# YonghaoHe/LFD-A-Light-and-Fast-Detector

Hardware: AMD Instinct MI355X
Metric: images/sec WIDERFACE-S 1920x1080 bs=8 end-to-end inference, LFD.precision='fp32_storage' (raw logits within 1e-4 of fp32: inside north_star's 1e-3; the 'fp16' mode, sigma 2.5e-3, under fp16_mode) (higher is better)
Workload: dtype f16

## Files before the change

### include/lfd_hip.h

```cpp
#ifndef LFD_HIP_H_
#define LFD_HIP_H_

#include <stddef.h>
#include <stdint.h>

#ifdef __cplusplus
extern "C" {
#endif

#define LFD_HIP_ABI_VERSION 3
#define LFD_MAX_LEVELS 8

typedef void* lfd_stream_t;

#if defined(LFD_BUILDING)
#define LFD_API __attribute__((visibility("default")))
#else
#define LFD_API
#endif

enum lfd_status {
  LFD_OK = 0,
  LFD_ERR_INVALID_ARGUMENT = -1,
  LFD_ERR_WORKSPACE_TOO_SMALL = -2,
// ... 204 lines not shown
                                              int32_t w, int32_t c, lfd_stream_t stream);
LFD_API int lfd_relu_inplace_f16(void* x, int64_t count, lfd_stream_t stream);
LFD_API int lfd_maxpool3x3s2_nhwc_f16(const void* in, void* out, int32_t n, int32_t h, int32_t w, int32_t c,
                                      lfd_stream_t stream);
LFD_API int lfd_pack_level_outputs_f32(const float* src, float* dst, int32_t n, int32_t hw, int32_t src_channels, int32_t c0,
                                       int32_t count, int32_t total_points, int32_t point_offset, float scale, int32_t op,
                                       lfd_stream_t stream);

LFD_API int lfd_conv2d_nhwc_f16_acc32(const lfd_conv_desc_t* desc, const void* in, float* out_f32, const void* w_packed,
                                      const float* bias, const void* zeros, lfd_stream_t stream);

typedef struct lfd_p32_conv_desc {
  int32_t n, h, w, cin, cout, ks, stride, relu;
  int32_t in_format;
  int32_t out_pixel_stride;
  int64_t out_image_stride;
} lfd_p32_conv_desc_t;
LFD_API size_t lfd_p32_conv_packed_weight_halfs(int32_t cin, int32_t cout, int32_t ks);
LFD_API int lfd_p32_conv2d_nhwc_f32(const lfd_p32_conv_desc_t* desc, const void* in, float* out, const void* w_packed,
                                    const float* bias, const float* residual, const float* scale, lfd_stream_t stream);
LFD_API int lfd_p32_conv2d_tail_nhwc_f32(const lfd_p32_conv_desc_t* desc, const void* in, float* out, const void* w_packed,
                                         const float* bias, const void* tail_w_packed, const float* tail_bias, int32_t tail_relu,
                                         lfd_stream_t stream);
LFD_API size_t lfd_p32_groupnorm_workspace_bytes(int32_t n, int32_t groups);
LFD_API int lfd_p32_groupnorm_relu_f32(float* x, int32_t n, int64_t hw, int32_t c, int32_t groups, const float* gamma,
                                       const float* beta, float eps, int32_t relu, void* workspace, size_t workspace_bytes,
                                       lfd_stream_t stream);

#define LFD_PL_GN_REPLICAS 8
typedef struct lfd_pl_conv_desc {
  int32_t n, h, w, cin, cout, ks, stride, relu;
  int32_t tail_cout, tail_relu;
  int32_t out_mode;
  int32_t f_c0, f_c1;
  float gn_in_eps;
  int64_t in_plane_halfs, out_plane_halfs, res_plane_halfs, ds_plane_halfs;
  int64_t f_image_stride0, f_image_stride1;
} lfd_pl_conv_desc_t;
LFD_API int lfd_pl_stem_pair(const void* in, int32_t in_format, int32_t n, int32_t h, int32_t w, int32_t channels,
                             const void* w1_packed, const float* b1, const void* w2_packed, const float* b2, void* out,
                             int64_t out_plane_halfs, lfd_stream_t stream);
LFD_API int lfd_pl_stem2x(const void* in, int32_t in_format, int32_t n, int32_t h, int32_t w, const void* w1_packed,
                          const void* w2_packed, const float* b2, const void* w3_packed, const float* b3,
                          const void* w4_packed, const float* b4, void* out, int64_t out_plane_halfs, const void* zeros,
                          lfd_stream_t stream);
LFD_API int lfd_pl_conv2d(const lfd_pl_conv_desc_t* desc, const void* in, void* out, const void* w_packed, const float* bias,
                          const void* residual, const void* tail_w_packed, const float* tail_bias, const void* ds_w_packed,
                          const float* ds_bias, void* ds_out, void* gn_sums, float* f_out0, float* f_out1, const float* scale1,
                          const void* gn_in_sums, const float* gn_in_gamma, const float* gn_in_beta, const void* zeros,
                          lfd_stream_t stream);
LFD_API int lfd_pl_block64(int32_t n, int32_t h, int32_t w, const void* in, int64_t in_plane_halfs, void* out,
                           int64_t out_plane_halfs, const void* w1_packed, const float* b1, const void* w2_packed,
                           const float* b2, const void* zeros, lfd_stream_t stream);
typedef struct lfd_pl_level {
  const void* in;
  void* out;
  const void* w_packed;
  const float* bias;
  const void* tail_w_packed;
  const float* tail_bias;
  void* gn_sums;
  const void* gn_in_sums;
  const float* gn_in_gamma;
  const float* gn_in_beta;
  float* f_out0;
  float* f_out1;
  const float* scale1;
  int32_t h, w;
  int64_t in_plane_halfs, out_plane_halfs;
} lfd_pl_level_t;
LFD_API int lfd_pl_conv2d_levels(const lfd_pl_conv_desc_t* desc, const lfd_pl_level_t* levels, int32_t num_levels,
                                 const void* zeros, lfd_stream_t stream);
LFD_API int lfd_pl_groupnorm_relu(void* x, int64_t plane_halfs, int32_t n, int64_t hw, int32_t c, const void* gn_sums,
                                  const float* gamma, const float* beta, float eps, int32_t relu, lfd_stream_t stream);

typedef struct lfd_pl_head_desc {
  int32_t mode, n, cin, relu0;
  int32_t f_c0, f_c1;
  float gn_in_eps;
  int32_t pad_;
  int64_t f_image_stride0, f_image_stride1;
} lfd_pl_head_desc_t;
typedef struct lfd_pl_head_level {
  const void* in;
  void* out;
  const void* w0;
  const float* b0;
  const void* w1;
  const float* b1;
  void* gn_sums;
  const void* gn_in_sums;
  const float* gn_in_gamma;
  const float* gn_in_beta;
  float* f_out0;
  float* f_out1;
  const float* scale1;
  int64_t in_plane_halfs;
  int32_t pixels, pad_;
} lfd_pl_head_level_t;
LFD_API int lfd_pl_head_levels(const lfd_pl_head_desc_t* desc, const lfd_pl_head_level_t* levels, int32_t num_levels,
                               const void* zeros, lfd_stream_t stream);

LFD_API int lfd_stem_conv_f16(const void* in, int32_t in_format, int32_t n, int32_t h, int32_t w,
                              int32_t channels, const void* w1_packed, const float* b1,
                              const void* w2_packed, const float* b2, void* out, lfd_stream_t stream);

// ... 232 lines not shown
```

### lfd-a-light-and-fast-detector_amd/lfd_amd/_lib.py

```python
import ctypes as C
import os

_HERE = os.path.dirname(os.path.abspath(__file__))
LIB_PATH = os.environ.get('LFD_HIP_LIB') or os.path.join(_HERE, 'liblfd_hip.so')
MAX_LEVELS = 8
F32, F16 = 0, 1

_lib = None


class DetectDesc(C.Structure):
    _fields_ = [('num_levels', C.c_int32),
                ('level_h', C.c_int32 * MAX_LEVELS), ('level_w', C.c_int32 * MAX_LEVELS),
                ('level_stride', C.c_int32 * MAX_LEVELS),
                ('level_range_lo', C.c_float * MAX_LEVELS), ('level_range_hi', C.c_float * MAX_LEVELS),
                ('num_classes', C.c_int32), ('num_cls_channels', C.c_int32),
                ('score_mode', C.c_int32), ('decode_mode', C.c_int32),
                ('class_agnostic', C.c_int32), ('max_candidates', C.c_int32),
                ('score_thr', C.c_float), ('iou_thr', C.c_float)]


class DetectExt(C.Structure):
    _fields_ = [('pre_nms_limit', C.c_int32), ('post_nms_limit', C.c_int32)]

# ... 175 lines not shown
    'lfd_gn_train_apply_f16': (C.c_int, [_P, _I32, _I64, _I32, _I32, _P, _P, _P, _I32, _P, _P]),
    'lfd_gn_train_stats_apply_f16': (C.c_int, [_P, _I32, _I64, _I32, _I32, _F, _P, _P, _I32, _P, _SZ, _P, _P, _P]),
    'lfd_gn_train_stats_apply_seg_f16': (C.c_int, [_P, _I32, _I32, _P, _I32, _I32, _F, _P, _P, _I32, _P, _SZ, _P, _P, _P]),
    'lfd_gn_train_bwd_seg_f16': (C.c_int, [_P, _P, _P, _I32, _I32, _P, _I32, _I32, _P, _P, _F, _I32, _P, _SZ, _P, _P, _P, _P]),
    'lfd_bn_train_apply_into_f16': (C.c_int, [_P, _I32, _I64, _I32, _P, _P, _P, _I32, _P, _I64, _I64, _P]),
    'lfd_bn_train_bwd_from_f16': (C.c_int, [_P, _I64, _I64, _P, _I32, _I32, _I64, _I32, _P, _P, _P, _F, _I32, _P, _SZ, _P, _P, _P, _P]),
    'lfd_head_out_split_concat_f16': (C.c_int, [_P, _I32, _I32, _I64, _I64, C.POINTER(HeadOutSeg), _I32, _P]),
    'lfd_head_out_grad_concat_f16': (C.c_int, [_P, _I32, _I32, _I64, _I64, C.POINTER(HeadOutSeg), _I32, _F, _P, _P, _SZ, _P]),
    'lfd_conv2d_bn_partials_nhwc_f16': (C.c_int, [C.POINTER(ConvDesc), _P, _P, _P, _P, _P, _P, _SZ, C.POINTER(C.c_int32), _P]),
    'lfd_bn_train_finish_into_levels_f16': (C.c_int, [C.POINTER(BnFwdLevel), _I32, _I32, _I32, _P, _I64, _P]),
    'lfd_bn_train_bwd_from_levels_f16': (C.c_int, [_P, _I64, C.POINTER(BnBwdLevel), _I32, _I32, _I32, _F, _I32, _P, _SZ, _P]),
    'lfd_head_out_split_levels_f16': (C.c_int, [_P, _I32, _I64, C.POINTER(HeadOutLevel), _I32, _P]),
    'lfd_head_out_grad_levels_f16': (C.c_int, [_P, _I32, _I64, C.POINTER(HeadOutLevel), _I32, _F, _P, _P, _SZ, _P]),
    'lfd_gn_train_bwd_f16': (C.c_int, [_P, _P, _P, _I32, _I64, _I32, _I32, _P, _P, _F, _I32, _P, _SZ, _P, _P, _P, _P]),
    'lfd_zero_insert2_nhwc_f16': (C.c_int, [_P, _I32, _I32, _I32, _I32, _I32, _I32, _P, _P]),
    'lfd_conv3x3s2_dgrad_nhwc_f16': (C.c_int, [_I32, _I32, _I32, _P, _P, _P, _P, _P]),
    'lfd_conv_wgrad_nhwc_f16': (C.c_int, [_P, _P, _I32, _I32, _I32, _I32, _I32, _I32, _I32, _F, _I32, _P, _SZ, _P, _P]),
    'lfd_conv_wgrad_partial_rows': (_I32, [_I32, _I32, _I32, _I32, _I32, _I32, _I32]),
    'lfd_conv_wgrad_partials_nhwc_f16': (C.c_int, [_P, _P, _I32, _I32, _I32, _I32, _I32, _I32, _I32, _P, _SZ, _P]),
    'lfd_conv1x1_wgrad_partials_of_bn_relu_f16': (C.c_int, [_P, _P, _P, _P, _P, _I32, _I32, _I32, _I32, _I32, _P, _SZ, _P]),
    'lfd_wgrad_final_batched_f32': (C.c_int, [_P, _I32, _I32, _P]),
    'lfd_rows_sum_batched_f32': (C.c_int, [_P, _I32, _P]),
    'lfd_stem_conv0_train_fwd': (C.c_int, [_P, _I32, _I32, _I32, _I32, _P, _P, _P]),
    'lfd_head_out_split_f16': (C.c_int, [_P, _I32, _I32, _I64, _I64, C.POINTER(HeadOutSeg), _I32, _P]),
    'lfd_head_out_grad_f16': (C.c_int, [_P, _I32, _I32, _I64, _I64, C.POINTER(HeadOutSeg), _I32, _F, _P, _P, _SZ, _P]),
    'lfd_stem_conv0_train_fwd_bn_stats': (C.c_int, [_P, _I32, _I32, _I32, _I32, _P, _P, _F, _F, _P, _P, _P, _SZ, _P, _P]),
    'lfd_stem_conv0_wgrad': (C.c_int, [_P, _P, _I32, _I32, _I32, _I32, _F, _I32, _P, _SZ, _P, _P]),
    'lfd_stem_conv0_bn_bwd_wgrad': (C.c_int, [_P, _P, _P, _I32, _I32, _I32, _I32, _P, _P, _P, _F, _I32, _P, _SZ, _P, _P, _P, _P]),
    'lfd_stem_conv0_bn_bwd_wgrad_rows': (C.c_int, [_P, _P, _P, _I32, _I32, _I32, _I32, _P, _P, _P, _F, _I32, _I32, _P, _SZ, _P, _P, _P, _P]),
    'lfd_bn_train_bwd_rows_f16': (C.c_int, [_P, _P, _I64, _I32, _P, _P, _P, _F, _I32, _I32, _P, _SZ, _P, _P, _P, _P]),
    'lfd_conv1x1_dgrad_bn_bwd_sums_nhwc_f16': (C.c_int, [C.POINTER(ConvDesc), _P, _P, _P, _P, _P, _P, _P, _P, _P, _P, _SZ, C.POINTER(C.c_int32), _P]),
    'lfd_stem_conv_f16': (C.c_int, [_P, _I32, _I32, _I32, _I32, _I32, _P, _P, _P, _P, _P, _P]),
    'lfd_stem_faster_fused_f16': (C.c_int, [_P, _I32, _I32, _I32, _I32, _I32, _P, _P, _P, _P, _P, _P, _P, _P, _P, _P]),
    'lfd_head_partial_floats': (_SZ, [C.POINTER(HeadDesc)]),
    'lfd_head_forward_f16': (C.c_int, [C.POINTER(HeadDesc), _I32, C.POINTER(HeadLevelPtrs), _P, _P, _P, _P, _P, _P, _P]),
    'lfd_head_forward_decode_f16': (C.c_int, [C.POINTER(HeadDesc), C.POINTER(HeadLevelPtrs), _P, _P, _P, _P, _P,
                                              C.POINTER(DetectDesc), _P, _P, _SZ, _P]),
    'lfd_groupnorm_finalize': (C.c_int, [C.POINTER(HeadDesc), _P, C.POINTER(C.c_void_p), C.POINTER(C.c_void_p), _F, _P, _P]),
    'lfd_groupnorm_finalize_fold': (C.c_int, [C.POINTER(HeadDesc), _P, C.POINTER(C.c_void_p), C.POINTER(C.c_void_p), _F, _P,
                                              C.POINTER(HeadLevelPtrs), _I32, _P]),
    'lfd_conv_packed_weight_halfs': (_SZ, [_I32, _I32, _I32]),
    'lfd_conv2d_nhwc_f16': (C.c_int, [C.POINTER(ConvDesc), _P, _P, _P, _P, _P, _P, _P, _P, _P]),
    'lfd_fasterblock_fused_f16': (C.c_int, [_I32, _I32, _I32, _P, _P, _P, _P, _P, _P, _P, _P]),
    'lfd_fasterblock128_fused_f16': (C.c_int, [_I32, _I32, _I32, _P, _P, _P, _P, _P, _P, _P]),
    'lfd_downblock_fused_f16': (C.c_int, [_I32, _I32, _I32, _P, _P, _P, _P, _P, _P, _P, _P, _P, _P]),
    'lfd_conv2d_nhwc_f16_acc32': (C.c_int, [C.POINTER(ConvDesc), _P, _P, _P, _P, _P, _P]),
    'lfd_p32_conv_packed_weight_halfs': (_SZ, [_I32, _I32, _I32]),
    'lfd_p32_conv2d_nhwc_f32': (C.c_int, [C.POINTER(P32ConvDesc), _P, _P, _P, _P, _P, _P, _P]),
    'lfd_p32_conv2d_tail_nhwc_f32': (C.c_int, [C.POINTER(P32ConvDesc), _P, _P, _P, _P, _P, _P, _I32, _P]),
    'lfd_pl_stem_pair': (C.c_int, [_P, _I32, _I32, _I32, _I32, _I32, _P, _P, _P, _P, _P, _I64, _P]),
    'lfd_pl_stem2x': (C.c_int, [_P, _I32, _I32, _I32, _I32, _P, _P, _P, _P, _P, _P, _P, _P, _I64, _P, _P]),
    'lfd_pl_conv2d': (C.c_int, [C.POINTER(PlConvDesc), _P, _P, _P, _P, _P, _P, _P, _P, _P, _P, _P, _P, _P, _P, _P, _P, _P, _P, _P]),
    'lfd_pl_block64': (C.c_int, [_I32, _I32, _I32, _P, _I64, _P, _I64, _P, _P, _P, _P, _P, _P]),
    'lfd_pl_conv2d_levels': (C.c_int, [C.POINTER(PlConvDesc), C.POINTER(PlLevel), _I32, _P, _P]),
    'lfd_pl_head_levels': (C.c_int, [C.POINTER(PlHeadDesc), C.POINTER(PlHeadLevel), _I32, _P, _P]),
    'lfd_pl_groupnorm_relu': (C.c_int, [_P, _I64, _I32, _I64, _I32, _P, _P, _P, _F, _I32, _P]),
    'lfd_p32_groupnorm_workspace_bytes': (_SZ, [_I32, _I32]),
    'lfd_p32_groupnorm_relu_f32': (C.c_int, [_P, _I32, _I64, _I32, _I32, _P, _P, _F, _I32, _P, _SZ, _P]),
    'lfd_conv2d_downsample_nhwc_f16': (C.c_int, [C.POINTER(ConvDesc), _P, _P, _P, _P, _P, _P, _P, _P, _P]),
}


TUNE_KEYS = {'HEAD2': 0, 'H2_CHUNK': 1, 'H2_AGPR': 2, 'H2_A1': 3, 'STEM2X': 4, 'X2_ALN': 5, 'X2_STAGGER': 6, 'BLOCK_ROWS': 7,
             'ROWS_WGS': 8, 'CONV128_SPLITK': 9, 'CONV0_VALU': 10, 'PL_C3': 11, 'PL_HEAD_OUT_REGS': 12, 'PL_HEAD_ROLES': 13, 'PL_STEM': 14}


def tune(name, value=None):
    key = TUNE_KEYS[name]
    prev = lib().lfd_tuning_get(key)
    if value is not None:
        check(lib().lfd_tuning_set(key, int(value)), 'lfd_tuning_set')
    return prev


def declared_symbols():
    return sorted(_SIGNATURES)


def lib():
    global _lib
    if _lib is None:
        if not os.path.exists(LIB_PATH):
            raise RuntimeError(
                'liblfd_hip.so not found at %s -- build it with `python __graft_entry__.py` '
                '(hipcc --offload-arch=gfx950); lfd_amd has no CPU/PyTorch fallback.' % LIB_PATH)
        import torch
        l = C.CDLL(LIB_PATH)
        for name, (res, args) in _SIGNATURES.items():
            fn = getattr(l, name)
            fn.restype, fn.argtypes = res, args
        if l.lfd_hip_abi_version() != ABI_VERSION:
            raise RuntimeError('liblfd_hip.so ABI version mismatch: %s reports %d, this package binds version %d '
                               '(struct layouts differ -- rebuild with `python __graft_entry__.py`)'
                               % (LIB_PATH, l.lfd_hip_abi_version(), ABI_VERSION))
        for name, key in TUNE_KEYS.items():
            v = os.environ.get('LFD_' + name)
            if v is not None and v.strip().lstrip('-').isdigit():
                l.lfd_tuning_set(key, int(v))
        _lib = l
    return _lib


def check(status, what):
    if status != 0:
        raise RuntimeError('%s failed: %s (status %d)' % (what, lib().lfd_hip_status_string(status).decode(), status))

# ... 15 lines not shown
```

### lfd-a-light-and-fast-detector_amd/lfd_amd/engine_p2.py

```python
import ctypes as C
import os

import torch
import torch.nn as nn

from . import _lib, engine, ops
from ._lib import check, lib, ptr, stream_ptr

_UNION = engine._UNION
_LO = 2048.0


class Unsupported(Exception):
    pass


def _split(w):
    w = w.detach().float()
    hi = w.half()
    lo = ((w - hi.float()) * _LO).half()
    return hi, lo


def pack_planes_weight(w):
# ... 5 lines not shown
    hi, lo = _split(w)
    return torch.stack([ops.pack_conv_weight(hi), ops.pack_conv_weight(lo)], 0).contiguous()


def pack_planes_stem_weight(w):
    hi, lo = _split(w)
    return torch.stack([engine.pack_stem_weight(hi), engine.pack_stem_weight(lo)], 0).contiguous()


def pack_planes_stem2x_weight(w, b):
    if tuple(w.shape) != (64, 3, 3, 3) or b.numel() != 64:
        raise Unsupported('fused stem: conv0 must be [64, 3, 3, 3]')
    c = 64
    wr = w.detach().float().permute(0, 2, 3, 1).reshape(c // 32, 32, 3, 9)
    out = torch.zeros(c // 32, 2, 2, 32, 8, dtype=torch.float32, device=w.device)
    out[:, 0, 0, :, 1:] = wr[:, :, 0, :7]
    out[:, 0, 1, :, 1:] = wr[:, :, 2, :7]
    out[:, 1, 0, :, 1:] = wr[:, :, 1, :7]
    for r in range(3):
        out[:, 1, 1, :, 2 * r:2 * r + 2] = wr[:, :, r, 7:9]
    out[:, 1, 1, :, 6] = b.detach().float().reshape(c // 32, 32).to(w.device)
    hi, lo = _split(out.reshape(c // 32, 2, 64, 8))
    return torch.stack([hi, lo], 0).contiguous()


def pack_planes_stem2x_tail_weight(w):
    if tuple(w.shape) != (64, 64, 1, 1):
        raise Unsupported('fused stem: first 1x1 must be [64, 64, 1, 1]')
    w2 = w.detach().float().reshape(64, 64)
    idx = torch.empty(4, 2, 8, dtype=torch.long)
    for q in range(4):
        s_, u = q // 2, q % 2
        for hh in range(2):
            for j in range(8):
                idx[q, hh, j] = 32 * s_ + 16 * u + (4 * hh + j if j < 4 else 8 + 4 * hh + j - 4)
    g = w2[:, idx.reshape(-1).to(w2.device)].reshape(2, 32, 4, 2, 8)
    out = g.permute(0, 2, 3, 1, 4).reshape(2, 4, 64, 8)
    hi, lo = _split(out)
    return torch.stack([hi, lo], 0).contiguous()


def _flat_head_enabled():
    return os.environ.get('LFD_P2_FLATHEAD', '1') != '0'


def _stem2x_enabled():
    return os.environ.get('LFD_P2_STEM2X', '1') != '0'


def _block_enabled():
    return os.environ.get('LFD_P2_BLOCK', '1') != '0'


def _pad_bias(b, mult=32):
    n = -(-b.numel() // mult) * mult
    out = b.new_zeros(n, dtype=torch.float32)
    out[:b.numel()] = b.float()
    return out


def to_planes(x):
    hi = x.half()
    return torch.stack([hi, ((x - hi.float()) * _LO).half()], 0).contiguous()


def from_planes(p):
    return p[0].float() + p[1].float() / _LO


_DISPATCH = {
    (64, 3, 1, 2): {'res'}, (64, 3, 2, 2): {'tail', 'ds'}, (64, 3, 2, 4): {'ds'}, (64, 1, 1, 4): {'tail', 'gn', 'out32'},
    (128, 3, 1, 4): {'res'}, (128, 3, 2, 4): {'ds'}, (128, 1, 1, 4): {'tail', 'gn', 'out32'}, (128, 1, 1, 1): {'out32'},
    (128, 1, 1, 2): {'out32'}, (32, 3, 2, 1): {'tail', 'ds'}, (32, 3, 2, 2): {'tail', 'ds'},
}


def _check_dispatch(cin, cout, ks, stride, tail, ds, res, gn, out32):
    opts = _DISPATCH.get((cin, ks, stride, -(-cout // 32)))
    used = {k for k, v in (('tail', tail), ('ds', ds), ('res', res), ('gn', gn), ('out32', out32)) if v}
    if opts is None or not (used - {'gn'} <= opts and (not gn or 'gn' in opts)) or len(used - {'gn'}) > 1:
        raise Unsupported('no plane kernel for conv %d -> %d k%d s%d %s' % (cin, cout, ks, stride, sorted(used)))
    if gn and (res or ds or out32):
        raise Unsupported('GroupNorm sums ride on a plain or chained 1x1')


def _fork_enabled():
    import os
    return os.environ.get('LFD_P2_FORK', '0') != '0'


def _levels_enabled():
    return os.environ.get('LFD_P2_LEVELS', '1') != '0'


class _Op(object):
    __slots__ = ('kind', 'src', 'dst', 'res', 'ds_dst', 'cin', 'cout', 'ks', 'stride', 'relu', 'w', 'b', 'tail', 'ds',
                 'out_mode', 'gn', 'gnin', 'level', 'f_c0', 'f_c1', 'scale', 'w1', 'b1', 'w2', 'b2', 'channels')

    def __init__(self, kind):
        self.kind = kind
        for k in self.__slots__[1:]:
            setattr(self, k, None)


class PlanesPlan(object):

    def __init__(self, model, device):
        self.device = device
        self.param_sig = engine._param_signature(model._backbone, model._neck, model._head)
        self._shape_cache = {}
        self.ops = []
        self.buf_channels = {}
        self.buf_scale = {}
        self._nbuf = 0
        self.num_gn = 0
        self.head_start = None
        self.level_ops = []
        self.tap_ready = []
        self.block_pairs = {}
        with torch.no_grad():
            self._build(model)

    def _new_buf(self, channels, scale):
        b = self._nbuf
        self._nbuf += 1
        self.buf_channels[b], self.buf_scale[b] = channels, scale
        return b

    def _conv(self, src, w, b, ks, stride, relu, res=None, tail=None, ds=None, gn=False, out32=None, gnin=None):
        dev = self.device
        cout, cin = w.shape[0], w.shape[1]
        if cin not in (32, 64, 128) or (out32 is None and cout % 32):
            raise Unsupported('conv %d -> %d' % (cin, cout))
        _check_dispatch(cin, cout, ks, stride, tail is not None, ds is not None, res is not None, gn, out32 is not None)
        o = _Op('conv')
        if gnin is not None:
            norm = gnin[1]
            if not (isinstance(norm, nn.GroupNorm) and norm.num_channels == 128 and norm.num_groups == 16 and cin == 128 and ks == 1
                    and stride == 1 and tail is None and res is None and ds is None):
                raise Unsupported('head norm must be GroupNorm(16, 128) in front of a 1x1 conv')
            o.gnin = (gnin[0], norm.weight.detach().float().contiguous().to(dev), norm.bias.detach().float().contiguous().to(dev),
                      float(norm.eps))
        o.src, o.res, o.ks, o.stride, o.relu, o.cin, o.cout = src, res, ks, stride, int(relu), cin, cout
        o.w = pack_planes_weight(w).to(dev)
        o.b = _pad_bias(b, 128).to(dev)
        sc = self.buf_scale[src] * stride
        if tail is not None:
            if tuple(tail[0].shape) != (cout, cout, 1, 1):
                raise Unsupported('chained 1x1 must be square')
            o.tail = (pack_planes_weight(tail[0]).to(dev), _pad_bias(tail[1], 128).to(dev), int(tail[2]))
        if ds is not None:
            if tuple(ds[0].shape) != (cout, cin, 1, 1) or ks != 3 or stride != 2:
                raise Unsupported('identity branch must be the 1x1 stride-2 twin of a 3x3 stride-2 conv')
            o.ds = (pack_planes_weight(ds[0]).to(dev), _pad_bias(ds[1], 128).to(dev))
            o.ds_dst = self._new_buf(cout, sc)
        if out32 is not None:
            o.out_mode = 2
            o.level, o.f_c0, o.f_c1, o.scale = out32
        else:
            o.out_mode = 1 if gn else 0
            o.dst = self._new_buf(cout, sc)
            if gn:
                if cout != 128:
                    raise Unsupported('GroupNorm sums: 128 channels in groups of 8')
                o.gn = self.num_gn
                self.num_gn += 1
        self.ops.append(o)
        return o

    def _build(self, model):
        bb, neck, head = model._backbone, model._neck, model._head
        if type(neck).__name__ != 'SimpleNeck' or type(head).__name__ != 'LFDHead':
            raise Unsupported('SimpleNeck + LFDHead')
        if bb._input_channels != 3 or (bb._norm_cfg is not None and bb._norm_cfg['type'] != 'BatchNorm2d'):
            raise Unsupported('backbone')
        for part in (bb, neck, head):
            for mod in part.modules():
                if not any(True for _ in mod.children()) and type(mod).__name__ not in (
                        'Conv2d', 'BatchNorm2d', 'GroupNorm', 'ReLU', 'Scale', 'Identity', 'Sequential', 'ModuleList'):
                    raise Unsupported('module %s (activation must be ReLU)' % type(mod).__name__)
        has_norm = bb._norm_cfg is not None
        step = 3 if has_norm else 2
        spec = list(bb.stem_spec())
        folded = [engine.fold_conv_norm(bb._stem[i * step], bb._stem[i * step + 1] if has_norm else None) for i in range(len(spec))]
        if len(spec) not in (2, 4) or [(k, s) for k, s, _, _ in spec] != [(3, 2), (1, 1)] * (len(spec) // 2):
            raise Unsupported('stem mode')
        c = folded[0][0].shape[0]
        if c not in (32, 64) or tuple(folded[1][0].shape[:2]) != (c, c):
            raise Unsupported('stem channels')
        o = _Op('stem')
        o.channels = c
        o.w1, o.b1 = pack_planes_stem_weight(folded[0][0]).to(self.device), _pad_bias(folded[0][1]).to(self.device)
        o.w2, o.b2 = pack_planes_weight(folded[1][0]).to(self.device), _pad_bias(folded[1][1]).to(self.device)
        o.dst = self._new_buf(c, 2)
        self.ops.append(o)
        cur = o.dst
        self.stem2x = None
        if len(spec) == 4:
            if tuple(folded[3][0].shape[:2]) != (c, c):
                raise Unsupported('stem channels')
            pair2 = self._conv(cur, folded[2][0], folded[2][1], 3, 2, True, tail=(folded[3][0], folded[3][1], True))
            cur = pair2.dst
            if c == 64:
                f = _Op('stem2x')
                f.w1 = pack_planes_stem2x_weight(folded[0][0], folded[0][1]).to(self.device)
                f.w2, f.b2 = pack_planes_stem2x_tail_weight(folded[1][0]).to(self.device), o.b2
                f.dst = cur
                f.tail = pair2
                self.stem2x = f
        taps = [tuple(t) for t in bb._out_indices]
        self.taps = []
        for i, nblk in enumerate(bb._body_architecture):
            for j in range(nblk):
                blk = getattr(bb, 'stage%d' % i)[j]
                ident, y = cur, cur
                for ci in range(1, blk.num_convs + 1):
                    conv = getattr(blk, '_conv%d' % ci)
                    w, b = engine.fold_conv_norm(conv, getattr(blk, '_norm%d' % ci, None))
                    ks, st = conv.kernel_size[0], conv.stride[0]
                    last = ci == blk.num_convs
                    ds = None
                    if ci == 1 and blk._downsample is not None:
                        dconv = blk._downsample[0]
                        if dconv.kernel_size[0] != 1 or dconv.stride[0] != 2 or (ks, st) != (3, 2) or last:
                            raise Unsupported('downsample branch')
                        ds = engine.fold_conv_norm(dconv, blk._downsample[1] if len(blk._downsample) > 1 else None)
                    elif ci > 1 and st != 1:
                        raise Unsupported('stride inside a block')
                    if ci == 1 and blk._downsample is None and st != 1:
                        raise Unsupported('strided block without a downsample branch')
                    op = self._conv(y, w, b, ks, st, True, res=ident if last else None, ds=ds)
                    if (ci == 2 and last and blk._downsample is None and self.ops[-2].dst == y and self.ops[-2].src == ident and
                            op.res == ident and
                            all(q.ks == 3 and q.stride == 1 and q.cin == 64 and q.cout == 64 and q.relu and q.tail is None
                                and q.ds is None and q.out_mode == 0 for q in self.ops[-2:])):
                        self.block_pairs[len(self.ops) - 2] = len(self.ops) - 1
                    y = op.dst
                    if ds is not None:
                        ident = op.ds_dst
                cur = y
                if (i, j) in taps:
                    self.taps.append(cur)
                    self.tap_ready.append(len(self.ops) - 1)
        if head._norm_cfg is None or head._conv_kernel_size != 1:
            raise Unsupported('head towers must be 1x1 conv + GroupNorm')
        nl = head._num_conv_layers
        union = head._regression_loss_type in _UNION
        self.cls_channels = head.num_cls_channels
        self.num_levels = head._num_heads
        ccls = self.cls_channels

        def tower(seq, t, first_tail_of=None):
            pend = None
            for l in range(nl):
                conv, norm = seq[l * 3], seq[l * 3 + 1]
                if not isinstance(norm, nn.GroupNorm):
                    raise Unsupported('head norm must be GroupNorm')
                if not isinstance(seq[l * 3 + 2], nn.ReLU):
                    raise Unsupported('head activation must be ReLU')
                bias = conv.bias.detach().float() if conv.bias is not None else torch.zeros(conv.out_channels, device=conv.weight.device)
                w = conv.weight.detach().float()
                if l == 0 and first_tail_of is not None:
                    nw, nb, src = first_tail_of
                    op = self._conv(src, nw, nb, 1, 1, True, tail=(w, bias, False), gn=True)
                else:
                    op = self._conv(t, w, bias, 1, 1, False, gn=True, gnin=pend)
                pend = (op.gn, norm)
                t = op.dst
            return t, pend

        self.head_start = len(self.ops)
        for i, f in enumerate(self.taps):
            first_op = len(self.ops)
            nseq = getattr(neck, 'neck%d' % i)
            nw, nb = engine.fold_conv_norm(nseq[0], nseq[1] if neck._norm_cfg is not None else None)
            if nw.shape[0] != 128 or nw.shape[2] != 1:
                raise Unsupported('neck must be 1x1 -> 128')
            cls_path = getattr(head, 'head%d_classification_path' % i)
            reg_path = getattr(head, 'head%d_regression_path' % i)
            scale = head._scales[i]._scale.detach().float().reshape(1).to(self.device) if union else None
            if head._merge_path_flag:
                if nl < 1:
                    raise Unsupported('merge path without tower convs')
                tt, pend = tower(getattr(head, 'head%d_merge_path' % i), None, first_tail_of=(nw, nb, f))
                cconv, rconv = cls_path[0], reg_path[0]
                if cconv.kernel_size[0] != 1 or rconv.kernel_size[0] != 1 or ccls + 4 > 64:
                    raise Unsupported('output convs')
                w = torch.cat([cconv.weight.detach().float(), rconv.weight.detach().float()], 0)
                b = torch.cat([cconv.bias.detach().float(), rconv.bias.detach().float()], 0)
# ... 160 lines not shown
                    if mode != 2:
                        lv.out, lv.gn_sums = st.bufs[o.dst].data_ptr(), st.gn_sums[o.gn].data_ptr()
                    if gi is not None:
                        lv.gn_in_sums, lv.gn_in_gamma, lv.gn_in_beta = st.gn_sums[gi[0]].data_ptr(), gi[1].data_ptr(), gi[2].data_ptr()
                        d.gn_in_eps = gi[3]
                    if mode == 2:
                        d.f_c0, d.f_c1 = o.f_c0, o.f_c1
                        d.f_image_stride0, d.f_image_stride1 = st.P * o.f_c0, st.P * 4
                        lv.f_out0 = (st.cls.data_ptr() + st.p_off[o.level] * o.f_c0 * 4) if o.f_c0 else None
                        lv.f_out1 = (st.reg.data_ptr() + st.p_off[o.level] * 4 * 4) if o.f_c1 else None
                        lv.scale1 = o.scale.data_ptr() if o.scale is not None else None
                calls.append((mode, d, arr, len(grp)))
            st.flat_calls = calls
        for mode, d, arr, n in st.flat_calls:
            if mode == 'G':
                check(l.lfd_pl_conv2d_levels(C.byref(d), arr, n, zeros, sp), 'lfd_pl_conv2d_levels')
            else:
                check(l.lfd_pl_head_levels(C.byref(d), arr, n, zeros, sp), 'lfd_pl_head_levels')

    def _launch_levels(self, st):
        modes = self._flat_head_modes() if _flat_head_enabled() else None
        if modes is not None:
            return self._launch_levels_flat(st, modes)
        l, sp = lib(), stream_ptr()
        zeros = ptr(ops.zero_line(self.device))
        if st.level_calls is None:
            calls = []
            for grp in self.level_groups:
                arr = (_lib.PlLevel * len(grp))()
                d0 = None
                for j, i in enumerate(grp):
                    o = self.ops[i]
                    d, src, dst, _, _, f0, f1 = self._desc(o, st)
                    d0 = d0 or d
                    lv, gi = arr[j], o.gnin
                    lv.in_, lv.out, lv.w_packed, lv.bias = src.data_ptr(), dst.data_ptr() if dst is not None else None, o.w.data_ptr(), o.b.data_ptr()
                    if o.tail is not None:
                        lv.tail_w_packed, lv.tail_bias = o.tail[0].data_ptr(), o.tail[1].data_ptr()
                    if o.gn is not None:
                        lv.gn_sums = st.gn_sums[o.gn].data_ptr()
                    if gi is not None:
                        lv.gn_in_sums, lv.gn_in_gamma, lv.gn_in_beta = st.gn_sums[gi[0]].data_ptr(), gi[1].data_ptr(), gi[2].data_ptr()
                    lv.f_out0, lv.f_out1 = f0, f1
                    lv.scale1 = o.scale.data_ptr() if o.scale is not None else None
                    lv.h, lv.w, lv.in_plane_halfs, lv.out_plane_halfs = src.shape[2], src.shape[3], d.in_plane_halfs, d.out_plane_halfs
                calls.append((d0, arr, len(grp)))
            st.level_calls = calls
        for d, arr, n in st.level_calls:
            check(l.lfd_pl_conv2d_levels(C.byref(d), arr, n, zeros, sp), 'lfd_pl_conv2d_levels')

    def _fused_block(self, st):
        return bool(self.block_pairs) and _block_enabled() and _lib.tune('PL_C3') == 2

    def _launch(self, x, fmt, st, indices):
        l, sp = lib(), stream_ptr()
        zeros = ptr(ops.zero_line(self.device))
        fblk = self._fused_block(st)
        blk_second = set(self.block_pairs.values()) if fblk else ()
        fused = (self.stem2x is not None and _stem2x_enabled() and
                 (os.environ.get('LFD_P2_STEM2X') == '2' or
                  (x.data_ptr() % 16 == 0 and ((fmt == 1 and st.w % 8 == 0) or (fmt == 2 and st.w % 16 == 0) or (fmt == 0 and st.w % 4 == 0)))))
        for i in indices:
            o = self.ops[i]
            if fblk:
                if i in blk_second:
                    continue
                j = self.block_pairs.get(i)
                if j is not None:
                    o2 = self.ops[j]
                    src, dst = st.bufs[o.src], st.bufs[o2.dst]
                    check(l.lfd_pl_block64(st.n, src.shape[2], src.shape[3], ptr(src), src[0].numel(), ptr(dst), dst[0].numel(),
                                           ptr(o.w), ptr(o.b), ptr(o2.w), ptr(o2.b), zeros, sp), 'lfd_pl_block64')
                    continue
            if fused and i < 2:
                if i == 0:
                    f, c2 = self.stem2x, self.stem2x.tail
                    dst = st.bufs[f.dst]
                    check(l.lfd_pl_stem2x(ptr(x), fmt, st.n, st.h, st.w, ptr(f.w1), ptr(f.w2), ptr(f.b2), ptr(c2.w), ptr(c2.b),
                                          ptr(c2.tail[0]), ptr(c2.tail[1]), ptr(dst), dst[0].numel(), zeros, sp), 'lfd_pl_stem2x')
                continue
            if o.kind == 'stem':
                dst = st.bufs[o.dst]
                check(l.lfd_pl_stem_pair(ptr(x), fmt, st.n, st.h, st.w, o.channels, ptr(o.w1), ptr(o.b1), ptr(o.w2), ptr(o.b2),
                                         ptr(dst), dst[0].numel(), sp), 'lfd_pl_stem_pair')
                continue
            d, src, dst, res, dsd, f0, f1 = self._desc(o, st)
            gi = o.gnin
            check(l.lfd_pl_conv2d(C.byref(d), ptr(src), ptr(dst), ptr(o.w), ptr(o.b), ptr(res),
                                  ptr(o.tail[0]) if o.tail else None, ptr(o.tail[1]) if o.tail else None,
                                  ptr(o.ds[0]) if o.ds else None, ptr(o.ds[1]) if o.ds else None, ptr(dsd),
                                  ptr(st.gn_sums[o.gn]) if o.gn is not None else None, f0, f1,
                                  ptr(o.scale) if o.scale is not None else None,
                                  ptr(st.gn_sums[gi[0]]) if gi else None, ptr(gi[1]) if gi else None, ptr(gi[2]) if gi else None,
                                  zeros, sp), 'lfd_pl_conv2d')


class _LazyBufs(dict):

    def __init__(self, st, plan):
        super().__init__()
        self._st, self._plan = st, plan

    def __missing__(self, b):
        hh, ww = self._st.dims[b]
        with torch.cuda.device(self._plan.device):
            t = torch.empty((2, self._st.n, hh, ww, self._plan.buf_channels[b]), dtype=torch.float16, device=self._plan.device)
        self[b] = t
        return t


class _State(object):

    def __init__(self, plan, n, h, w):
        dev = plan.device
        self.n, self.h, self.w = n, h, w
        self.dims = {}
# ... 22 lines not shown
```

Baseline: 6638.

## Fuse stride-2 downsample residual block into one LDS-pipelined planes kernel

Adds a fused kernel for the 64-channel downsampling residual block: conv1 (3x3 stride 2), the 1x1 downsample branch, and conv2 (3x3) with the residual add all run in one launch. Two waves produce the intermediate and identity rows into LDS rings, and two more waves consume them with a row lag, so neither intermediate is written to or read back from global memory. The residual add is done through identity-matrix MFMAs. It is on by default for large enough feature maps. The cost is one workgroup per CU, because of heavy LDS use and large register weight caches, plus added complexity in synchronisation.

Result: faster. 6743, median of 6 (+1.6%).

```diff
diff --git a/include/lfd_hip.h b/include/lfd_hip.h
--- a/include/lfd_hip.h
+++ b/include/lfd_hip.h
@@ -280,6 +280,9 @@
 LFD_API int lfd_pl_block64(int32_t n, int32_t h, int32_t w, const void* in, int64_t in_plane_halfs, void* out,
                            int64_t out_plane_halfs, const void* w1_packed, const float* b1, const void* w2_packed,
                            const float* b2, const void* zeros, lfd_stream_t stream);
+LFD_API int lfd_pl_down64(int32_t n, int32_t h, int32_t w, const void* in, int64_t in_plane_halfs, void* out,
+                          int64_t out_plane_halfs, const void* w1_packed, const float* b1, const void* wds_packed,
+                          const float* bds, const void* w2_packed, const float* b2, const void* zeros, lfd_stream_t stream);
 typedef struct lfd_pl_level {
   const void* in;
   void* out;
diff --git a/lfd-a-light-and-fast-detector_amd/csrc/planes_down.hip b/lfd-a-light-and-fast-detector_amd/csrc/planes_down.hip
--- /dev/null
+++ b/lfd-a-light-and-fast-detector_amd/csrc/planes_down.hip
@@ -0,0 +1,390 @@
+#include "planes_impl.h"
+
+namespace pl {
+namespace {
+
+struct DnArgs {
+  const _Float16* in;
+  long in_plane;
+  _Float16* out;
+  long out_plane;
+  const half8* w1;
+  const float* b1;
+  const half8* wd;
+  const float* bd;
+  const half8* w2;
+  const float* b2;
+  const _Float16* zeros;
+  int N, H, W, OH, OW;
+  int strips, segs, SH, nwork;
+};
+
+struct DN {
+  static constexpr int TW = 30;
+  static constexpr int IW = 65, MW = 34, DW = 32;
+  static constexpr int NDMA = 9;
+  static constexpr int IN_PLANE = IW * 128, IN_SLOT = 2 * IN_PLANE, NIN = 6;
+  static constexpr int MID_PLANE = MW * 128, MID_SLOT = 2 * MID_PLANE, NMID = 4;
+  static constexpr int ID_PLANE = DW * 128, ID_SLOT = 2 * ID_PLANE, NID = 3;
+  static constexpr int NK = 36, NQ = 4, KA = 18;
+  static constexpr int LAG = 3;
+  static constexpr int OFF_IN = 0;
+  static constexpr int OFF_MID = OFF_IN + NIN * IN_SLOT;
+  static constexpr int OFF_ID = OFF_MID + NMID * MID_SLOT;
+  static constexpr int OFF_BIAS = OFF_ID + NID * ID_SLOT;
+  static constexpr int LDS_BYTES = OFF_BIAS + 3 * 64 * 4;
+};
+static_assert(DN::LDS_BYTES <= 160 * 1024, "LDS capacity");
+static_assert(DN::NIN >= 6 && DN::NMID >= 4 && DN::NID >= 3, "ring depths (see the header)");
+
+struct DSeg { int n, oy0, ox0, R; };
+
+struct DnRow {
+  const char* rowp;
+  char* lrow;
+  bool rv;
+};
+
+__device__ __forceinline__ DnRow dn_row(const DnArgs& a, char* smem, const DSeg& sg, int plane, int ir) {
+  DnRow r;
+  const int gy = 2 * sg.oy0 - 3 + ir;
+  r.rv = gy >= 0 && gy < a.H && ir <= 2 * sg.R + 4;
+  r.rowp = reinterpret_cast<const char*>(a.in + (size_t)plane * a.in_plane) + ((long)sg.n * a.H + (r.rv ? gy : 0)) * (long)a.W * 128;
+  r.lrow = smem + DN::OFF_IN + (ir % DN::NIN) * DN::IN_SLOT + plane * DN::IN_PLANE;
+  return r;
+}
+
+__device__ __forceinline__ void dn_dma(const DnArgs& a, const DSeg& sg, const DnRow& r, int i) {
+  const int L = threadIdx.x & 63;
+  const int p = 8 * i + (L >> 3);
+  const int c = (L & 7) ^ ((p >> 1) & 7);
+  const int gx = 2 * sg.ox0 - 3 + p;
+  const bool ok = r.rv && gx >= 0 && gx < a.W;
+  const char* src = ok ? r.rowp + (long)gx * 128 + c * 16 : reinterpret_cast<const char*>(a.zeros) + c * 16;
+  if (i < DN::NDMA - 1 || L < 8) dma16(src, r.lrow + i * 1024);
+}
+
+__device__ __forceinline__ void dn_dma_all(const DnArgs& a, const DSeg& sg, const DnRow& r) {
+#pragma unroll
+  for (int i = 0; i < DN::NDMA; ++i) dn_dma(a, sg, r, i);
+}
+
+__device__ __forceinline__ half8 dn_identity_fragment(int pix, int h, int qq) {
+  int j0 = pix - 16 * qq - 8 * h;
+  asm volatile("" : "+v"(j0));
+  union { half8 v; uint32_t u[4]; } f;
+#pragma unroll
+  for (int r = 0; r < 4; ++r) f.u[r] = (j0 == 2 * r) ? 0x3c00u : ((j0 == 2 * r + 1) ? 0x3c000000u : 0u);
+  return f.v;
+}
+
+__device__ __forceinline__ void bias_init(f32x16& m, f32x16& c, const float* bp) {
+#pragma unroll
+  for (int g = 0; g < 4; ++g) {
+    const float4 b4 = *reinterpret_cast<const float4*>(bp + 8 * g);
+    m[4 * g + 0] = b4.x; m[4 * g + 1] = b4.y; m[4 * g + 2] = b4.z; m[4 * g + 3] = b4.w;
+  }
+#pragma unroll
+  for (int r = 0; r < 16; ++r) c[r] = 0.f;
+}
+
+__device__ __forceinline__ void dn_conv1(const DnArgs& a, char* smem, int ct, const DSeg& sg) {
+  const int lane = threadIdx.x & 63;
+  const int h = lane >> 5, pix = lane & 31;
+  const int T = sg.R + DN::LAG;
+  dn_dma_all(a, sg, dn_row(a, smem, sg, ct, 0));
+  dn_dma_all(a, sg, dn_row(a, smem, sg, ct, 2));
+  half8 wh[DN::NK], wl[DN::NK], wdh[DN::NQ], wdl[DN::NQ];
+  {
+    const half8* wsrc = a.w1 + (size_t)(ct * DN::NK) * 64 + lane;
+    constexpr long WPL = 2L * DN::NK * 64;
+#pragma unroll
+    for (int k = 0; k < DN::NK; ++k) {
+      wh[k] = wsrc[(size_t)k * 64];
+      wl[k] = wsrc[WPL + (size_t)k * 64];
+    }
+    const half8* dsrc = a.wd + (size_t)(ct * DN::NQ) * 64 + lane;
+    constexpr long DPL = 2L * DN::NQ * 64;
+#pragma unroll
+    for (int q = 0; q < DN::NQ; ++q) {
+      wdh[q] = dsrc[(size_t)q * 64];
+      wdl[q] = dsrc[DPL + (size_t)q * 64];
+    }
+  }
+  const float* sb = reinterpret_cast<const float*>(smem + DN::OFF_BIAS);
+  int xoff[3][DN::NQ];
+#pragma unroll
+  for (int s = 0; s < 3; ++s) {
+    const int p = 2 * pix + s;
+#pragma unroll
+    for (int q = 0; q < DN::NQ; ++q) xoff[s][q] = p * 128 + (((2 * q + h) ^ ((p >> 1) & 7)) * 16);
+  }
+  const char* ring = smem + DN::OFF_IN;
+  const int my_base = sg.oy0 - 1, mx = sg.ox0 - 1 + pix;
+  const bool col_in = mx >= 0 && mx < a.OW;
+  const int wsw = pix & 7;
+
+  block_barrier();
+  for (int j = 0; j < T; ++j) {
+    asm volatile("s_waitcnt vmcnt(0)" ::: "memory");
+    block_barrier();
+    const DnRow dr = dn_row(a, smem, sg, ct, 2 * j + 4);
+    if (j < sg.R + 2) {
+      f32x16 accm, accc, adm, adc;
+      bias_init(accm, accc, sb + ct * 32 + 4 * h);
+      bias_init(adm, adc, sb + 64 + ct * 32 + 4 * h);
+      int rb[3];
+#pragma unroll
+      for (int r = 0; r < 3; ++r) rb[r] = ((2 * j + r) % DN::NIN) * DN::IN_SLOT;
+      auto xaddr = [&](int k) {
+        const int r = k / 12, s = (k / 4) % 3, q = k % 4;
+        return ring + rb[r] + xoff[s][q];
+      };
+      constexpr int PD = 3;
+      half8 xqh[PD + 1], xql[PD + 1];
+#pragma unroll
+      for (int k = 0; k < PD; ++k) {
+        const char* p = xaddr(k);
+        xqh[k] = *reinterpret_cast<const half8*>(p);
+        xql[k] = *reinterpret_cast<const half8*>(p + DN::IN_PLANE);
+      }
+      static_for([&](auto kc) {
+        constexpr int k = decltype(kc)::value;
+        if constexpr (k % 4 == 1 && k / 4 < DN::NDMA) dn_dma(a, sg, dr, k / 4);
+        if constexpr (k + PD < DN::NK) {
+          const char* p = xaddr(k + PD);
+          xqh[(k + PD) % (PD + 1)] = *reinterpret_cast<const half8*>(p);
+          xql[(k + PD) % (PD + 1)] = *reinterpret_cast<const half8*>(p + DN::IN_PLANE);
+        }
+        PL_SB();
+        accm = __builtin_amdgcn_mfma_f32_32x32x16_f16(wh[k], xqh[k % (PD + 1)], accm, 0, 0, 0);
+        accc = __builtin_amdgcn_mfma_f32_32x32x16_f16(wh[k], xql[k % (PD + 1)], accc, 0, 0, 0);
+        accc = __builtin_amdgcn_mfma_f32_32x32x16_f16(wl[k], xqh[k % (PD + 1)], accc, 0, 0, 0);
+        if constexpr (k / 4 == 4) {
+          adm = __builtin_amdgcn_mfma_f32_32x32x16_f16(wdh[k % 4], xqh[k % (PD + 1)], adm, 0, 0, 0);
+          adc = __builtin_amdgcn_mfma_f32_32x32x16_f16(wdh[k % 4], xql[k % (PD + 1)], adc, 0, 0, 0);
+          adc = __builtin_amdgcn_mfma_f32_32x32x16_f16(wdl[k % 4], xqh[k % (PD + 1)], adc, 0, 0, 0);
+        }
+        PL_SB();
+      }, std::make_integer_sequence<int, DN::NK>{});
+      const int my = my_base + j;
+      const bool inimg = col_in && my >= 0 && my < a.OH;
+      char* mid = smem + DN::OFF_MID + (j % DN::NMID) * DN::MID_SLOT + pix * 128 + h * 8;
+      char* idp = smem + DN::OFF_ID + (j % DN::NID) * DN::ID_SLOT + pix * 128 + h * 8;
+#pragma unroll
+      for (int g = 0; g < 4; ++g) {
+        const int o = ((4 * ct + g) ^ wsw) * 16;
+        float y[4], d[4];
+#pragma unroll
+        for (int e = 0; e < 4; ++e) {
+          y[e] = fmaxf(comb(accm[4 * g + e], accc[4 * g + e]), 0.f);
+          d[e] = comb(adm[4 * g + e], adc[4 * g + e]);
+        }
+        uint2 vh, vl, dh, dl;
+        split2(y[0], y[1], vh.x, vl.x);
+        split2(y[2], y[3], vh.y, vl.y);
+        split2(d[0], d[1], dh.x, dl.x);
+        split2(d[2], d[3], dh.y, dl.y);
+        if (!inimg) { vh = uint2{0u, 0u}; vl = uint2{0u, 0u}; }
+        *reinterpret_cast<uint2*>(mid + o) = vh;
+        *reinterpret_cast<uint2*>(mid + DN::MID_PLANE + o) = vl;
+        *reinterpret_cast<uint2*>(idp + o) = dh;
+        *reinterpret_cast<uint2*>(idp + DN::ID_PLANE + o) = dl;
+      }
+    } else {
+      dn_dma_all(a, sg, dr);
+    }
+  }
+}
+
+__device__ __forceinline__ void dn_conv2(const DnArgs& a, char* smem, int ct, const DSeg& sg) {
+  const int lane = threadIdx.x & 63;
+  const int h = lane >> 5, pix = lane & 31;
+  const int T = sg.R + DN::LAG;
+  dn_dma_all(a, sg, dn_row(a, smem, sg, ct, 1));
+  dn_dma_all(a, sg, dn_row(a, smem, sg, ct, 3));
+  half8 wh[DN::NK], wl[DN::NK];
+  {
+    const half8* wsrc = a.w2 + (size_t)(ct * DN::NK) * 64 + lane;
+    constexpr long WPL = 2L * DN::NK * 64;
+#pragma unroll
+    for (int k = 0; k < DN::NK; ++k) {
+      wh[k] = wsrc[(size_t)k * 64];
+      wl[k] = wsrc[WPL + (size_t)k * 64];
+    }
+  }
+  const float* sb = reinterpret_cast<const float*>(smem + DN::OFF_BIAS) + 128;
+  int xoff[3][DN::NQ];
+#pragma unroll
+  for (int s = 0; s < 3; ++s) {
+    const int p = pix + s;
+#pragma unroll
+    for (int q = 0; q < DN::NQ; ++q) xoff[s][q] = p * 128 + (((2 * q + h) ^ (p & 7)) * 16);
+  }
+  const char* ring = smem + DN::OFF_MID;
+  const int ox = sg.ox0 + pix;
+  const bool col_out = pix < DN::TW && ox < a.OW;
+  _Float16* const obase = a.out + ct * 32 + 4 * h;
+  uint32_t eh[8], el[8];
+#pragma unroll
+  for (int r = 0; r < 8; ++r) eh[r] = el[r] = 0u;
+  auto store_row = [&](int ol) {
+    if (col_out) {
+      _Float16* o = obase + (((size_t)sg.n * a.OH + sg.oy0 + ol) * a.OW + ox) * 64;
+#pragma unroll
+      for (int g = 0; g < 4; ++g) {
+        *reinterpret_cast<uint2*>(o + 8 * g) = uint2{eh[2 * g], eh[2 * g + 1]};
+        *reinterpret_cast<uint2*>(o + a.out_plane + 8 * g) = uint2{el[2 * g], el[2 * g + 1]};
+      }
+    }
+  };
+
+  block_barrier();
+  for (int j = 0; j < T; ++j) {
+    asm volatile("s_waitcnt vmcnt(%0)" ::"n"(DN::NDMA) : "memory");
+    block_barrier();
+    const int olp = j - 1 - DN::LAG;
+    if (olp >= 0 && olp < sg.R) store_row(olp);
+    const DnRow dr = dn_row(a, smem, sg, ct, 2 * j + 5);
+    const int ol = j - DN::LAG;
+    if (ol >= 0 && ol < sg.R) {
+      f32x16 am, ac, bm, bc;
+      bias_init(am, ac, sb + ct * 32 + 4 * h);
+#pragma unroll
+      for (int r = 0; r < 16; ++r) bm[r] = bc[r] = 0.f;
+      int rb[3];
+#pragma unroll
+      for (int r = 0; r < 3; ++r) rb[r] = ((ol + r) % DN::NMID) * DN::MID_SLOT;
+      auto xaddr = [&](int k) {
+        const int r = k / 12, s = (k / 4) % 3, q = k % 4;
+        return ring + rb[r] + xoff[s][q];
+      };
+      constexpr int PD = 3;
+      half8 xqh[PD + 1], xql[PD + 1];
+#pragma unroll
+      for (int k = 0; k < PD; ++k) {
+        const char* p = xaddr(k);
+        xqh[k] = *reinterpret_cast<const half8*>(p);
+        xql[k] = *reinterpret_cast<const half8*>(p + DN::MID_PLANE);
+      }
+      static_for([&](auto kc) {
+        constexpr int k = decltype(kc)::value;
+        if constexpr (k % 4 == 1 && k / 4 < DN::NDMA) dn_dma(a, sg, dr, k / 4);
+        if constexpr (k + PD < DN::NK) {
+          const char* p = xaddr(k + PD);
+          xqh[(k + PD) % (PD + 1)] = *reinterpret_cast<const half8*>(p);
+          xql[(k + PD) % (PD + 1)] = *reinterpret_cast<const half8*>(p + DN::MID_PLANE);
+        }
+        PL_SB();
+        if constexpr (k < DN::KA) {
+          am = __builtin_amdgcn_mfma_f32_32x32x16_f16(wh[k], xqh[k % (PD + 1)], am, 0, 0, 0);
+          ac = __builtin_amdgcn_mfma_f32_32x32x16_f16(wh[k], xql[k % (PD + 1)], ac, 0, 0, 0);
+          ac = __builtin_amdgcn_mfma_f32_32x32x16_f16(wl[k], xqh[k % (PD + 1)], ac, 0, 0, 0);
+        } else {
+          bm = __builtin_amdgcn_mfma_f32_32x32x16_f16(wh[k], xqh[k % (PD + 1)], bm, 0, 0, 0);
+          bc = __builtin_amdgcn_mfma_f32_32x32x16_f16(wh[k], xql[k % (PD + 1)], bc, 0, 0, 0);
+          bc = __builtin_amdgcn_mfma_f32_32x32x16_f16(wl[k], xqh[k % (PD + 1)], bc, 0, 0, 0);
+        }
+        PL_SB();
+        if constexpr (k == DN::KA - 1) {
+          const int ip = pix < 31 ? pix + 1 : 31;
+          const char* ib = smem + DN::OFF_ID + ((ol + 1) % DN::NID) * DN::ID_SLOT + ip * 128;
+#pragma unroll
+          for (int qq = 0; qq < 2; ++qq) {
+            const int o = ((4 * ct + 2 * qq + h) ^ (ip & 7)) * 16;
+            const half8 rh = *reinterpret_cast<const half8*>(ib + o);
+            const half8 rl = *reinterpret_cast<const half8*>(ib + DN::ID_PLANE + o);
+            const half8 idf = dn_identity_fragment(pix, h, qq);
+            am = __builtin_amdgcn_mfma_f32_32x32x16_f16(idf, rh, am, 0, 0, 0);
+            ac = __builtin_amdgcn_mfma_f32_32x32x16_f16(idf, rl, ac, 0, 0, 0);
+          }
+        }
+      }, std::make_integer_sequence<int, DN::NK>{});
+#pragma unroll
+      for (int g = 0; g < 4; ++g) {
+        float y[4];
+#pragma unroll
+        for (int e = 0; e < 4; ++e) y[e] = fmaxf(comb(bm[4 * g + e], bc[4 * g + e]) + comb(am[4 * g + e], ac[4 * g + e]), 0.f);
+        split2(y[0], y[1], eh[2 * g], el[2 * g]);
+        split2(y[2], y[3], eh[2 * g + 1], el[2 * g + 1]);
+      }
+    } else {
+      dn_dma_all(a, sg, dr);
+    }
+  }
+  if (sg.R >= 1) store_row(sg.R - 1);
+}
+
+__global__ __launch_bounds__(256, 1) void k_pl_down64(DnArgs a) {
+  extern __shared__ __attribute__((aligned(16))) char smem[];
+  const int wave = __builtin_amdgcn_readfirstlane((int)(threadIdx.x >> 6));
+  if (threadIdx.x < 192) {
+    float* sb = reinterpret_cast<float*>(smem + DN::OFF_BIAS);
+    const int t = threadIdx.x;
+    sb[t] = t < 64 ? a.b1[t] : (t < 128 ? a.bd[t - 64] : a.b2[t - 128]);
+  }
+  const int w = blockIdx.x;
+  DSeg sg;
+  {
+    const int per_img = a.segs * a.strips;
+    sg.n = w / per_img;
+    const int r = w - sg.n * per_img;
+    const int seg = r / a.strips, strip = r - seg * a.strips;
+    sg.oy0 = seg * a.SH;
+    sg.ox0 = strip * DN::TW;
+    sg.R = (a.OH - sg.oy0) < a.SH ? (a.OH - sg.oy0) : a.SH;
+  }
+  if (wave < 2) dn_conv1(a, smem, wave, sg);
+  else dn_conv2(a, smem, wave - 2, sg);
+}
+
+}
+}
+
+extern "C" LFD_API int lfd_pl_down64(int32_t n, int32_t h, int32_t w, const void* in, int64_t in_plane_halfs, void* out,
+                                     int64_t out_plane_halfs, const void* w1_packed, const float* b1, const void* wds_packed,
+                                     const float* bds, const void* w2_packed, const float* b2, const void* zeros,
+                                     lfd_stream_t stream) {
+  if (!in || !out || !w1_packed || !b1 || !wds_packed || !bds || !w2_packed || !b2 || !zeros) return LFD_ERR_INVALID_ARGUMENT;
+  if (n < 1 || h < 1 || w < 1) return LFD_ERR_INVALID_ARGUMENT;
+  if (!lfd_aligned16(in) || !lfd_aligned16(out) || !lfd_aligned16(w1_packed) || !lfd_aligned16(wds_packed) ||
+      !lfd_aligned16(w2_packed))
+    return LFD_ERR_INVALID_ARGUMENT;
+  const int oh = (h + 1) / 2, ow = (w + 1) / 2;
+  const long in_pl = (long)n * h * w * 64, out_pl = (long)n * oh * ow * 64;
+  if (in_plane_halfs < in_pl || out_plane_halfs < out_pl || (in_plane_halfs & 7) || (out_plane_halfs & 7))
+    return LFD_ERR_INVALID_ARGUMENT;
+  const char *ib = (const char*)in, *ob = (const char*)out;
+  if (ib < ob + 2 * out_plane_halfs * 2 && ob < ib + 2 * in_plane_halfs * 2) return LFD_ERR_INVALID_ARGUMENT;
+  pl::DnArgs a{};
+  a.in = (const _Float16*)in; a.in_plane = in_plane_halfs;
+  a.out = (_Float16*)out; a.out_plane = out_plane_halfs;
+  a.w1 = (const half8*)w1_packed; a.b1 = b1;
+  a.wd = (const half8*)wds_packed; a.bd = bds;
+  a.w2 = (const half8*)w2_packed; a.b2 = b2;
+  a.zeros = (const _Float16*)zeros;
+  a.N = n; a.H = h; a.W = w; a.OH = oh; a.OW = ow;
+  static unsigned long long attr_done_mask = 0;
+  const int dev = lfd_device_ordinal();
+  if (LFD_ONCE_PER_DEVICE(attr_done_mask, dev)) {
+    if (hipFuncSetAttribute(reinterpret_cast<const void*>(&pl::k_pl_down64), hipFuncAttributeMaxDynamicSharedMemorySize,
+                            pl::DN::LDS_BYTES) != hipSuccess)
+      return LFD_ERR_LAUNCH_FAILED;
+    LFD_DONE_ON_DEVICE(attr_done_mask, dev);
+  }
+  a.strips = (ow + pl::DN::TW - 1) / pl::DN::TW;
+  const long cols = (long)n * a.strips;
+  int segs = (int)(256 / cols);
+  if (segs < 1) segs = 1;
+  int sh = (oh + segs - 1) / segs;
+  if (sh < 4) sh = 4;
+  if (sh > oh) sh = oh;
+  a.SH = sh;
+  a.segs = (oh + sh - 1) / sh;
+  const long nwork = cols * a.segs;
+  if (nwork > 0x7fffffffL) return LFD_ERR_UNSUPPORTED;
+  a.nwork = (int)nwork;
+  hipLaunchKernelGGL(pl::k_pl_down64, dim3(a.nwork), dim3(256), pl::DN::LDS_BYTES, (hipStream_t)stream, a);
+  LFD_CHECK_LAUNCH();
+  return LFD_OK;
+}
diff --git a/lfd-a-light-and-fast-detector_amd/lfd_amd/_lib.py b/lfd-a-light-and-fast-detector_amd/lfd_amd/_lib.py
--- a/lfd-a-light-and-fast-detector_amd/lfd_amd/_lib.py
+++ b/lfd-a-light-and-fast-detector_amd/lfd_amd/_lib.py
@@ -251,6 +251,7 @@
     'lfd_pl_stem2x': (C.c_int, [_P, _I32, _I32, _I32, _I32, _P, _P, _P, _P, _P, _P, _P, _P, _I64, _P, _P]),
     'lfd_pl_conv2d': (C.c_int, [C.POINTER(PlConvDesc), _P, _P, _P, _P, _P, _P, _P, _P, _P, _P, _P, _P, _P, _P, _P, _P, _P, _P, _P]),
     'lfd_pl_block64': (C.c_int, [_I32, _I32, _I32, _P, _I64, _P, _I64, _P, _P, _P, _P, _P, _P]),
+    'lfd_pl_down64': (C.c_int, [_I32, _I32, _I32, _P, _I64, _P, _I64, _P, _P, _P, _P, _P, _P, _P, _P]),
     'lfd_pl_conv2d_levels': (C.c_int, [C.POINTER(PlConvDesc), C.POINTER(PlLevel), _I32, _P, _P]),
     'lfd_pl_head_levels': (C.c_int, [C.POINTER(PlHeadDesc), C.POINTER(PlHeadLevel), _I32, _P, _P]),
     'lfd_pl_groupnorm_relu': (C.c_int, [_P, _I64, _I32, _I64, _I32, _P, _P, _P, _F, _I32, _P]),
diff --git a/lfd-a-light-and-fast-detector_amd/lfd_amd/engine_p2.py b/lfd-a-light-and-fast-detector_amd/lfd_amd/engine_p2.py
--- a/lfd-a-light-and-fast-detector_amd/lfd_amd/engine_p2.py
+++ b/lfd-a-light-and-fast-detector_amd/lfd_amd/engine_p2.py
@@ -81,6 +81,13 @@
     return os.environ.get('LFD_P2_BLOCK', '1') != '0'
 
 
+def _down_mode():
+    return os.environ.get('LFD_P2_DOWN', '1')
+
+
+_DOWN_MIN_PIXELS = 12288
+
+
 def _pad_bias(b, mult=32):
     n = -(-b.numel() // mult) * mult
     out = b.new_zeros(n, dtype=torch.float32)
@@ -147,6 +154,7 @@
         self.level_ops = []
         self.tap_ready = []
         self.block_pairs = {}
+        self.down_pairs = {}
         with torch.no_grad():
             self._build(model)
 
@@ -243,6 +251,7 @@
             for j in range(nblk):
                 blk = getattr(bb, 'stage%d' % i)[j]
                 ident, y = cur, cur
+                ident_in = cur
                 for ci in range(1, blk.num_convs + 1):
                     conv = getattr(blk, '_conv%d' % ci)
                     w, b = engine.fold_conv_norm(conv, getattr(blk, '_norm%d' % ci, None))
@@ -264,6 +273,13 @@
                             all(q.ks == 3 and q.stride == 1 and q.cin == 64 and q.cout == 64 and q.relu and q.tail is None
                                 and q.ds is None and q.out_mode == 0 for q in self.ops[-2:])):
                         self.block_pairs[len(self.ops) - 2] = len(self.ops) - 1
+                    if ci == 2 and last and blk._downsample is not None:
+                        o1 = self.ops[-2]
+                        if (o1.src == ident_in and o1.dst == y and o1.ds is not None and op.res == o1.ds_dst and
+                                o1.ks == 3 and o1.stride == 2 and op.ks == 3 and op.stride == 1 and
+                                all(q.cin == 64 and q.cout == 64 and q.relu and q.tail is None and q.out_mode == 0
+                                    for q in (o1, op)) and op.ds is None):
+                            self.down_pairs[len(self.ops) - 2] = len(self.ops) - 1
                     y = op.dst
                     if ds is not None:
                         ident = op.ds_dst
@@ -530,16 +546,36 @@
     def _fused_block(self, st):
         return bool(self.block_pairs) and _block_enabled() and _lib.tune('PL_C3') == 2
 
+    def _fused_down(self, st):
+        mode = _down_mode()
+        if not self.down_pairs or mode == '0' or _lib.tune('PL_C3') != 2:
+            return {}
+        return {i: j for i, j in self.down_pairs.items()
+                if mode == '2' or st.n * st.dims[self.ops[j].dst][0] * st.dims[self.ops[j].dst][1] >= _DOWN_MIN_PIXELS}
+
     def _launch(self, x, fmt, st, indices):
         l, sp = lib(), stream_ptr()
         zeros = ptr(ops.zero_line(self.device))
         fblk = self._fused_block(st)
         blk_second = set(self.block_pairs.values()) if fblk else ()
+        fdown = self._fused_down(st)
+        down_second = set(fdown.values())
         fused = (self.stem2x is not None and _stem2x_enabled() and
                  (os.environ.get('LFD_P2_STEM2X') == '2' or
                   (x.data_ptr() % 16 == 0 and ((fmt == 1 and st.w % 8 == 0) or (fmt == 2 and st.w % 16 == 0) or (fmt == 0 and st.w % 4 == 0)))))
         for i in indices:
             o = self.ops[i]
+            if fdown:
+                if i in down_second:
+                    continue
+                j = fdown.get(i)
+                if j is not None:
+                    o2 = self.ops[j]
+                    src, dst = st.bufs[o.src], st.bufs[o2.dst]
+                    check(l.lfd_pl_down64(st.n, src.shape[2], src.shape[3], ptr(src), src[0].numel(), ptr(dst), dst[0].numel(),
+                                          ptr(o.w), ptr(o.b), ptr(o.ds[0]), ptr(o.ds[1]), ptr(o2.w), ptr(o2.b), zeros, sp),
+                          'lfd_pl_down64')
+                    continue
             if fblk:
                 if i in blk_second:
                     continue
```
